# sandeep06011991/OCC-GNN

Measured on AMD Instinct MI355X. Metric: sampled_edges_per_sec, higher is better.
Workload: dtype u32; 1 GPU; products-like synthetic (N=2449029, mean degree 50.5, pareto degrees, seed 0), GraphSAGE fanout 15/10/5 (layer 0 = seeds' hop), minibatch 1024, 4 parts (v % 4), engine-only (sample+slice); streams=128, round_overlap=True, device_lists=int32 (host exports widen to the reference's int64), engine_device_bytes=16549793524

## Files before the change

occ-gnn_amd/csrc/cslicer_hip.hip:

```cpp
#include <hip/hip_runtime.h>

#include <cstdarg>
#include <cstdio>
#include <cstdlib>
#include <cstring>
#include <algorithm>
#include <deque>
#include <vector>

#include "cslicer_hip.h"

namespace {

constexpr uint32_t UNSET = 0xFFFFFFFFu;

constexpr int TN = 256;
#ifdef CSL_OCC7
#define CSL_LB256 __launch_bounds__(256)
#else
#define CSL_LB256 __launch_bounds__(256, 8)
#endif
constexpr int CSL_MAX_SETS = 4;
constexpr int NW = TN / 64;
#ifndef CSL_TPB
#define CSL_TPB 4
#endif
#ifndef CSL_HLOG
#define CSL_HLOG 12
#endif
#ifndef CSL_QMEAN
#define CSL_QMEAN 2048
#endif
#ifndef CSL_SCT
#define CSL_SCT 4096
#endif
#ifndef CSL_SU
#define CSL_SU 1
#endif
constexpr int TPB = CSL_TPB;
constexpr int HLOG = CSL_HLOG;
constexpr int HCAP = 1 << HLOG;
constexpr int QMEAN = CSL_QMEAN;
constexpr int SCT = CSL_SCT;
constexpr int DEG_BITS = 24;
constexpr uint32_t DEG_MASK = (1u << DEG_BITS) - 1;

constexpr int K_NEED = 0;
constexpr int K_EDGES = 1;
constexpr int K_NEWF = 2;
__host__ __device__ constexpr int K_IN(int P, int g) { return 3 + g; }
__host__ __device__ constexpr int K_OUT(int P, int g) { return 3 + P + g; }
__host__ __device__ constexpr int K_OWNED(int P, int g) { return 3 + 2 * P + g; }
__host__ __device__ constexpr int K_SELF(int P, int g) { return 3 + 3 * P + g; }
__host__ __device__ constexpr int K_TO(int P, int g) { return 3 + 4 * P + g; }
__host__ __device__ constexpr int K_FROM(int P, int g) { return 3 + 5 * P + g; }
__host__ __device__ constexpr int K_ECNT(int P, int g) { return 3 + 6 * P + g; }
__host__ __device__ constexpr int K_PAIR(int P, int g, int p) { return 3 + 7 * P + g * P + p; }
__host__ __device__ constexpr int NKINDS(int P, bool graph) { return graph ? 3 + 7 * P + P * P : 3 + 6 * P; }
constexpr int MAXK = 3 + 7 * CSL_MAX_PARTS + CSL_MAX_PARTS * CSL_MAX_PARTS;

enum { KN_SEEDS = 0, KN_DEGREE, KN_SCAN_A, KN_SAMPLE, KN_SCAN_Q, KN_SCATTER, KN_BUCKET, KN_COUNT, KN_SCAN_B,
       KN_EMIT, KN_SELFIN, KN_MT, KN_EDGES, KN_DUPSEEDS, KN_SELFIN_DEGREE };
const char* const kKernelNames[CSL_NUM_KERNELS] = {"k_seeds",   "k_degree", "k_scan_need", "k_sample",
                                                   "k_scan_buckets", "k_scatter", "k_bucket", "k_count",
                                                   "k_scan_lists", "k_emit",  "k_selfin",  "k_mt19937_fill",
                                                   "k_graph", "k_dupseeds", "k_selfin_degree"};

struct LArgs {
  const unsigned long long* rowinfo;
  const uint32_t* off32;
  const uint32_t* indices;
  const uint8_t* wl;
  uint32_t N, P;
  const uint32_t* ring;
  unsigned long long ring_mask, gen_lo, gen_hi;
  unsigned long long* rngpos;
  unsigned long long* rngbase;
  unsigned long long* acc;
  const uint32_t* fr_in;
  uint32_t* fr_out;
  size_t fr_in_stride, fr_out_stride;
  uint32_t fr_out_cap;
  unsigned long long* ninfo;
  uint32_t* hasedge;
  uint32_t* selfpos;
  uint32_t* firstpos;
  size_t fcap;
  uint32_t* cand;
  uint8_t* cflag;
  uint32_t* crank;
  uint2* queue;
  size_t ccap;
  uint32_t* nbk;
  uint32_t* bcnt;
  uint32_t* bcur;
  uint32_t nbmax;
  uint32_t* tcnt;
  uint32_t tmax, nk;
  uint32_t* fsize;
  csl_sample_meta* meta;
  int* arena;
  size_t arena_stride;
  size_t list_base[CSL_NUM_LISTS];
  uint32_t layer, fanout, W;
  unsigned long long wmagic;
  uint32_t S;
  uint32_t tpb;
  uint32_t* boff;
  uint32_t* ticket;
  uint32_t pmagic;
  uint32_t pmask;
  uint32_t last;
  uint32_t* dupflag;
  uint32_t* seedrep;
  uint32_t* dupfirst;
  uint32_t* dupout;
  size_t fcap0;
  unsigned long long* rngend;
  uint32_t* candk;
  uint32_t graph;
  uint8_t* ecnt;
  uint32_t* srcpos;
  uint32_t* tcur;
};

constexpr uint32_t SELF_BIT = 0x80000000u;
constexpr int kNoReplaceMaxFanout = 64;

__device__ __forceinline__ uint32_t mod_parts(const LArgs& a, uint32_t v) {
  uint32_t r = v - __umulhi(v, a.pmagic) * a.P;
  if (r >= a.P) r -= a.P;
  if (r >= a.P) r -= a.P;
  return r;
}
__device__ __forceinline__ uint32_t owner(const LArgs& a, uint32_t v) {
  return a.wl ? (uint32_t)a.wl[v] : mod_parts(a, v);
}
__device__ __forceinline__ unsigned long long row_lookup(const LArgs& a, uint32_t v) {
  if (a.off32) {
    const uint32_t lo = a.off32[v], hi = a.off32[v + 1];
    return ((unsigned long long)lo << 24) | (unsigned long long)(hi - lo);
  }
  return a.rowinfo[v];
}
__device__ __forceinline__ uint32_t lane_id() { return threadIdx.x & 63; }
__device__ __forceinline__ uint32_t div_w(const LArgs& a, uint32_t c) {
  return (uint32_t)(((unsigned long long)c * a.wmagic) >> 40);
}
__device__ __forceinline__ bool xcd_block_at(const LArgs& a, uint32_t id, uint32_t grid, uint32_t& x, uint32_t& s) {
  const uint32_t groups = (a.S + 7u) >> 3;
  const uint32_t per_stream = grid / (8u * groups);
  const uint32_t j = id >> 3;
  const uint32_t sl = j / per_stream;
  x = j - sl * per_stream;
  s = sl * 8u + (id & 7u);
  return s < a.S;
}
__device__ __forceinline__ bool xcd_block(const LArgs& a, uint32_t& x, uint32_t& s) {
  return xcd_block_at(a, blockIdx.x, gridDim.x, x, s);
}
__device__ __forceinline__ void st_sc1(uint32_t* p, uint32_t v) {
  __hip_atomic_store(p, v, __ATOMIC_RELAXED, __HIP_MEMORY_SCOPE_AGENT);
}
__device__ __forceinline__ uint32_t ld_sc1(const uint32_t* p) {
  return __hip_atomic_load(p, __ATOMIC_RELAXED, __HIP_MEMORY_SCOPE_AGENT);
}
__device__ __forceinline__ bool last_block_of_stream(uint32_t* ticket, uint32_t expected) {
  __shared__ uint32_t s_last;
  asm volatile("s_waitcnt vmcnt(0)" ::: "memory");
  __syncthreads();
  if (threadIdx.x == 0) {
    const uint32_t t = __hip_atomic_fetch_add(ticket, 1u, __ATOMIC_RELAXED, __HIP_MEMORY_SCOPE_AGENT);
    s_last = t == expected - 1u;
    if (t == expected - 1u) {
      st_sc1(ticket, 0u);
      __builtin_amdgcn_fence(__ATOMIC_ACQUIRE, "agent");
      asm volatile("s_waitcnt vmcnt(0)" ::: "memory");
    }
  }
  __syncthreads();
  return s_last != 0u;
}
__device__ __forceinline__ unsigned long long lt_mask() {
  return (1ull << lane_id()) - 1ull;
}
__device__ __forceinline__ uint32_t bucket_of(uint32_t v, uint32_t nb) {
  return __umulhi(v * 0x9E3779B1u, nb);
}
__device__ __forceinline__ uint32_t pass_of(uint32_t v, uint32_t npass) {
  uint32_t x = v * 0x27D4EB2Fu;
  x ^= x >> 13;
  return __umulhi(x * 0x165667B1u, npass);
}
__device__ __forceinline__ uint32_t slot_of(uint32_t v) {
  uint32_t x = v * 0x85EBCA6Bu;
  x ^= x >> 15;
  x *= 0xC2B2AE35u;
  return x >> (32 - HLOG);
}

__device__ __forceinline__ uint32_t wave_excl_scan(uint32_t x, uint32_t& total) {
  uint32_t incl = x;
  for (int o = 1; o < 64; o <<= 1) {
    uint32_t y = __shfl_up(incl, o);
    if ((int)lane_id() >= o) incl += y;
  }
  total = __shfl(incl, 63);
  return incl - x;
}

__device__ __forceinline__ uint32_t wave_incl_scan_dpp(uint32_t x) {
  int v = (int)x;
  v += __builtin_amdgcn_update_dpp(0, v, 0x111, 0xf, 0xf, false);
  v += __builtin_amdgcn_update_dpp(0, v, 0x112, 0xf, 0xf, false);
  v += __builtin_amdgcn_update_dpp(0, v, 0x114, 0xf, 0xf, false);
  v += __builtin_amdgcn_update_dpp(0, v, 0x118, 0xf, 0xf, false);
  v += __builtin_amdgcn_update_dpp(0, v, 0x142, 0xa, 0xf, false);
  v += __builtin_amdgcn_update_dpp(0, v, 0x143, 0xc, 0xf, false);
  return (uint32_t)v;
}
__device__ __forceinline__ uint32_t spread4(uint32_t x) { return ((x & 0xFu) * 0x00204081u) & 0x01010101u; }

constexpr int SCAN_CH = 12;

template <int PHASE>
__device__ __forceinline__ void scan_body(const LArgs& a, const int s) {
  const uint32_t F = ld_sc1(&a.fsize[s * (CSL_MAX_LAYERS + 1) + a.layer]);
  const uint32_t ntiles = (F + TN - 1) / TN;
  const int k_lo = PHASE == 0 ? 0 : 2;
  const int k_hi = PHASE == 0 ? 2 : (int)a.nk;
  __shared__ uint32_t s_tot[MAXK];
  const int w = threadIdx.x >> 6, nw = blockDim.x >> 6;
  const uint32_t chunk = (ntiles + 63) / 64;
  for (int k = k_lo + w; k < k_hi; k += nw) {
    uint32_t* p = a.tcnt + ((size_t)s * a.nk + k) * a.tmax;
    if (chunk <= (uint32_t)SCAN_CH) {
      const uint32_t t0 = lane_id() * chunk;
      uint32_t x[SCAN_CH], sum = 0;
#pragma unroll
      for (int j = 0; j < SCAN_CH; j++) {
        x[j] = ((uint32_t)j < chunk && t0 + j < ntiles) ? ld_sc1(&p[t0 + j]) : 0u;
        sum += x[j];
      }
      uint32_t tot;
      uint32_t run = wave_excl_scan(sum, tot);
#pragma unroll
      for (int j = 0; j < SCAN_CH; j++) {
        if ((uint32_t)j < chunk && t0 + j < ntiles) p[t0 + j] = run;
        run += x[j];
      }
      if (lane_id() == 0) s_tot[k] = tot;
    } else {
      uint32_t run = 0;
      for (uint32_t t0 = 0; t0 < ntiles; t0 += 64) {
        const uint32_t t = t0 + lane_id();
        const uint32_t x = t < ntiles ? ld_sc1(&p[t]) : 0;
        uint32_t tot;
        const uint32_t ex = wave_excl_scan(x, tot);
        if (t < ntiles) p[t] = run + ex;
        run += tot;
      }
      if (lane_id() == 0) s_tot[k] = run;
    }
  }
  if (PHASE == 0) {
    const unsigned long long C = (unsigned long long)F * a.W;
    uint32_t nb = (uint32_t)((C + QMEAN - 1) / QMEAN);
    if (nb < 1) nb = 1;
    if (nb > a.nbmax) nb = a.nbmax;
    if (threadIdx.x == 0) a.nbk[s] = F ? nb : 0;
    for (uint32_t b = threadIdx.x; b <= a.nbmax; b += blockDim.x) {
      a.bcnt[(size_t)s * (a.nbmax + 1) + b] = 0;
      if (b < a.nbmax) a.bcur[(size_t)s * a.nbmax + b] = 0;
    }
  }
  __syncthreads();
  csl_layer_meta& m = a.meta[s].layer[a.layer];
  if (PHASE == 0) {
    if (threadIdx.x == 0) {
      const unsigned long long base = a.rngpos[s];
      const unsigned long long draws = (unsigned long long)s_tot[K_NEED] * a.fanout;
      a.rngbase[s] = base;
      a.rngpos[s] = base + draws;
      a.rngend[s] = base + draws;
      if (a.layer == 0) a.meta[s].rng_begin = base;
      a.meta[s].rng_end = base + draws;
      a.acc[2 * s] += s_tot[K_EDGES];
      if (a.layer == 0 && F) a.acc[2 * s + 1] += 1;
      m.frontier = F;
      m.draws = (uint32_t)draws;
      m.sampled_edges = s_tot[K_EDGES];
    }
  } else {
    const int P = (int)a.P;
    const uint32_t t = threadIdx.x;
    auto pair_sum = [&](int g, bool from) -> uint32_t {
      uint32_t x = 0;
      for (int p = 0; p < P; p++) x += from ? s_tot[K_PAIR(P, g, p)] : s_tot[K_PAIR(P, p, g)];
      return x;
    };
    auto tot_of = [&](int kind, int g) -> uint32_t {
      switch (kind) {
        case CSL_IN_NODES: return s_tot[K_IN(P, g)];
        case CSL_OUT_NODES: return s_tot[K_OUT(P, g)];
        case CSL_OWNED_OUT_NODES: return s_tot[K_OWNED(P, g)];
        case CSL_SELF_IDS_IN:
        case CSL_SELF_IDS_OUT: return s_tot[K_SELF(P, g)];
        case CSL_TO_IDS: return a.graph ? pair_sum(g, false) : s_tot[K_TO(P, g)];
        case CSL_FROM_IDS: return a.graph ? pair_sum(g, true) : s_tot[K_FROM(P, g)];
        case CSL_INDPTR: return a.graph ? (F ? s_tot[K_OUT(P, g)] + 1 : 0u) : 0u;
        case CSL_INDICES: return a.graph ? s_tot[K_ECNT(P, g)] : 0u;
        case CSL_T_INDPTR: return a.tcur ? (F ? s_tot[K_IN(P, g)] + 1 : 0u) : 0u;
        case CSL_T_INDICES: return a.tcur ? s_tot[K_ECNT(P, g)] + s_tot[K_SELF(P, g)] : 0u;
        default: return a.graph ? s_tot[K_OWNED(P, g)] : 0u;
      }
    };
    if (t < (uint32_t)CSL_NUM_LISTS) {
      uint32_t run = 0;
      for (int g = 0; g < P; g++) {
        m.off[t][g] = run;
        run += tot_of((int)t, g);
      }
      for (int g = P; g <= CSL_MAX_PARTS; g++) m.off[t][g] = run;
    } else if (t == 16) {
      uint32_t nf = s_tot[K_NEWF];
      if (nf > a.fr_out_cap) {
        atomicOr(&a.meta[s].error, (uint32_t)CSL_ERR_FRONTIER_CAP);
        nf = a.fr_out_cap;
      }
      m.next_frontier = nf;
      a.fsize[s * (CSL_MAX_LAYERS + 1) + a.layer + 1] = nf;
    } else if (t == 17) {
      for (int g = 0; g < CSL_MAX_PARTS; g++)
        m.indptr_len[g] = g < P ? tot_of(a.graph ? CSL_INDPTR : CSL_OUT_NODES, g) : 0u;
    } else if (a.graph && t >= 32 && t < 32u + (uint32_t)P) {
      const int g = (int)t - 32;
      uint32_t fr = 0, to = 0;
      for (int p = 0; p < P; p++) {
        m.pair_off[0][g][p] = fr;
        m.pair_off[1][g][p] = to;
        fr += s_tot[K_PAIR(P, g, p)];
        to += s_tot[K_PAIR(P, p, g)];
      }
      for (int p = P; p <= CSL_MAX_PARTS; p++) {
        m.pair_off[0][g][p] = fr;
        m.pair_off[1][g][p] = to;
      }
    }
  }
}

struct BatchDesc {
  long long offset;
  int count;
  int pad;
};

__device__ __forceinline__ void degree_body(const LArgs& a, const uint32_t bx, const uint32_t s, const uint32_t per_stream,
                                            const long long* __restrict__ nodes, const BatchDesc* __restrict__ desc) {
  uint32_t F;
  long long noff = 0;
  if (a.layer == 0) {
    const BatchDesc d = desc[s];
    F = (uint32_t)d.count;
    noff = d.offset;
    if (bx == 0 && threadIdx.x == 0) {
      st_sc1(&a.fsize[s * (CSL_MAX_LAYERS + 1)], F);
      for (uint32_t l = 1; l <= CSL_MAX_LAYERS; l++) a.fsize[s * (CSL_MAX_LAYERS + 1) + l] = 0;
      a.dupflag[s] = 0;
      a.meta[s].n_seeds = F;
    }
  } else {
    F = a.fsize[s * (CSL_MAX_LAYERS + 1) + a.layer];
  }
  const uint32_t tile = bx * NW + (threadIdx.x >> 6);
  if (tile * TN < F) {
    const uint32_t i0 = tile * TN + lane_id() * 4;
    unsigned long long ri[4] = {0, 0, 0, 0};
    if (a.layer == 0) {
      uint32_t v[4];
#pragma unroll
      for (int j = 0; j < 4; j++) {
        v[j] = UNSET;
        if (i0 + j < F) {
          long long id = nodes[noff + i0 + j];
          if (id < 0 || id >= (long long)a.N) {
            atomicOr(&a.meta[s].error, (uint32_t)CSL_ERR_SEED_RANGE);
            id = 0;
          }
          v[j] = (uint32_t)id;
        }
      }
#pragma unroll
      for (int j = 0; j < 4; j++)
        if (v[j] != UNSET) ri[j] = row_lookup(a, v[j]);
#pragma unroll
      for (int j = 0; j < 4; j++) {
        if (v[j] != UNSET) {
          const_cast<uint32_t*>(a.fr_in)[s * a.fr_in_stride + i0 + j] = v[j];
          a.ninfo[s * a.fcap + i0 + j] = ri[j];
        }
      }
    } else {
#pragma unroll
      for (int j = 0; j < 4; j++)
        if (i0 + j < F) ri[j] = a.ninfo[s * a.fcap + i0 + j];
    }
    uint32_t need = 0, ne = 0;
#pragma unroll
    for (int j = 0; j < 4; j++) {
      if (i0 + j < F) {
        const uint32_t deg = (uint32_t)(ri[j] & DEG_MASK);
        need += deg >= a.fanout;
        ne += deg < a.fanout ? deg : a.fanout;
      }
    }
    for (int o = 32; o > 0; o >>= 1) {
      need += __shfl_down(need, o);
      ne += __shfl_down(ne, o);
    }
    if (lane_id() == 0) {
      st_sc1(&a.tcnt[((size_t)s * a.nk + K_NEED) * a.tmax + tile], need);
      st_sc1(&a.tcnt[((size_t)s * a.nk + K_EDGES) * a.tmax + tile], ne);
    }
  }
  uint32_t nb_act = ((F + TN - 1) / TN + NW - 1) / NW;
  if (nb_act < 1) nb_act = 1;
  if (nb_act > per_stream) nb_act = per_stream;
  if (bx >= nb_act) return;
  if (last_block_of_stream(a.ticket + 2 * s, nb_act)) scan_body<0>(a, (int)s);
}

__global__ CSL_LB256 void k_degree(LArgs a, const long long* __restrict__ nodes,
                                               const BatchDesc* __restrict__ desc) {
  uint32_t bx, s;
  if (!xcd_block(a, bx, s)) return;
  degree_body(a, bx, s, gridDim.x / (8u * ((a.S + 7u) >> 3)), nodes, desc);
}

__device__ __forceinline__ uint32_t mt_temper(uint32_t y) {
  y ^= y >> 11;
  y ^= (y << 7) & 0x9d2c5680u;
  y ^= (y << 15) & 0xefc60000u;
  y ^= y >> 18;
  return y;
}

__device__ __forceinline__ uint32_t ring_word(const LArgs& a, uint32_t s, unsigned long long pos) {
  if (pos >= a.gen_lo && pos < a.gen_hi) return a.ring[pos & a.ring_mask];
  atomicOr(&a.meta[s].error, (uint32_t)CSL_ERR_RNG_WINDOW);
  return 0;
}
__device__ __forceinline__ uint32_t floyd_pick(const LArgs& a, uint32_t s, unsigned long long row_pos, uint32_t j,
                                               uint32_t D, uint32_t rj) {
  uint32_t x = rj % (D + j + 1u);
  const uint32_t own = x;
  uint32_t m = j;
  bool taken = false;
  for (;;) {
    for (uint32_t i = 0; i < m; i++) {
      if (ring_word(a, s, row_pos + i) % (D + i + 1u) == x) taken = true;
    }
    if (taken || x < D || x - D >= m) break;
    m = x - D;
    x = ring_word(a, s, row_pos + m) % (D + m + 1u);
  }
  return taken ? D + j : own;
}

__global__ CSL_LB256 void k_sample(LArgs a) {
  constexpr bool NOREP = false;
  constexpr bool WEIGHTED = false;
  constexpr const uint32_t* cum = nullptr;
#include "k_sample_body.inc"
}
__global__ CSL_LB256 void k_sample_norep(LArgs a) {
  constexpr bool NOREP = true;
  constexpr bool WEIGHTED = false;
  constexpr const uint32_t* cum = nullptr;
#include "k_sample_body.inc"
}
__global__ CSL_LB256 void k_sample_weighted(LArgs a, const uint32_t* __restrict__ cum) {
  constexpr bool NOREP = false;
  constexpr bool WEIGHTED = true;
#include "k_sample_body.inc"
}

__global__ __launch_bounds__(256) void k_check_cdf(const unsigned long long* __restrict__ rowinfo,
// ... 127 lines not shown
  const uint32_t staged = s_loff[nb - 1] + s_hist[nb - 1];
  for (uint32_t k = n; k < staged; k += TN) {
    const uint2 e = s_stage[k];
    const uint32_t b = bucket_of(e.x, nb);
    q[s_gbase[b] + (k - s_loff[b])] = e;
  }
}

__device__ __forceinline__ uint32_t ht_find(const uint32_t* h_key, uint32_t val) {
  uint32_t h = slot_of(val);
  for (uint32_t probes = 0; probes < (uint32_t)HCAP; probes++) {
    const uint32_t k = h_key[h];
    if (k == val) return h;
    if (k == UNSET) return UNSET;
    h = (h + 1) & (HCAP - 1);
  }
  return UNSET;
}

#ifndef CSL_BT
#define CSL_BT 512
#endif
#ifndef CSL_RC
#define CSL_RC 4
#endif
constexpr int BT = CSL_BT;
constexpr int RC = CSL_RC;

__device__ __forceinline__ uint32_t ht_insert(uint32_t* h_key, uint32_t val) {
  uint32_t h = slot_of(val);
  for (uint32_t probes = 0; probes < (uint32_t)HCAP; probes++) {
    uint32_t kk = h_key[h];
    if (kk == UNSET) kk = atomicCAS(&h_key[h], UNSET, val);
    if (kk == UNSET || kk == val) return h;
    h = (h + 1) & (HCAP - 1);
  }
  return UNSET;
}

#ifndef CSL_BPB
#define CSL_BPB 4
#endif
constexpr int BPB = CSL_BPB;

__device__ unsigned long long g_wave_dup[3];

template <bool HAS_WL, bool PROBE = false>
__global__ __launch_bounds__(BT) void k_bucket(LArgs a) {
  uint32_t bx, s;
  if (!xcd_block(a, bx, s)) return;
  const uint32_t nbk = a.nbk[s];
  uint32_t b = bx * BPB;
  if (b >= nbk) return;
  __shared__ __attribute__((aligned(16))) uint32_t h_key[HCAP];
  __shared__ __attribute__((aligned(16))) uint32_t h_epos[HCAP];
  __shared__ __attribute__((aligned(16))) uint32_t h_self[HCAP];
  const uint32_t n = threadIdx.x;
  const uint32_t* off = a.boff + (size_t)s * (a.nbmax + 1);
  const uint2* qs = a.queue + (size_t)s * a.ccap;
  const uint32_t W = a.W;
  uint32_t q0 = off[b], q1 = off[b + 1];
  uint2 e[RC];
#pragma unroll
  for (int r = 0; r < RC; r++) e[r] = n + r * BT < q1 - q0 ? qs[q0 + n + r * BT] : make_uint2(UNSET, 0u);
  auto record = [&](const uint2 ee, const uint32_t h) {
    if (ee.y & SELF_BIT) {
      atomicMin(&h_self[h], ee.y & ~SELF_BIT);
      if (a.graph) atomicMin(&h_epos[h], (ee.y & ~SELF_BIT) * W);
    } else {
      atomicMin(&h_epos[h], ee.y);
    }
  };
  auto insert = [&](const uint2 ee) -> uint32_t {
    const uint32_t h = ht_insert(h_key, ee.x);
    if (h == UNSET) {
      atomicOr(&a.meta[s].error, (uint32_t)CSL_ERR_BUCKET_FULL);
    } else {
      record(ee, h);
    }
    return h;
  };
  uint8_t* cflag = a.cflag + (size_t)s * a.ccap;
  auto part_of = [&](const uint32_t v) -> uint32_t { return HAS_WL ? (uint32_t)a.wl[v] : mod_parts(a, v); };
  auto judge = [&](const uint2 ee, const uint32_t epos, const uint32_t self, const uint32_t g) {
    if (ee.y & SELF_BIT) {
      const uint32_t i = ee.y & ~SELF_BIT;
      const uint32_t c = i * W;
      if (self != i) {
        if (a.graph) atomicOr(&a.meta[s].error, (uint32_t)CSL_ERR_DUP_SEED);
        else a.dupflag[s] = 1u;
      }
      if (a.graph) {
        const uint32_t fe = epos == c;
        if (!fe) cflag[c] = 0;
        a.firstpos[s * a.fcap + i] = epos;
      } else {
        const uint32_t newf = epos > c && self == i;
        if (!newf) cflag[c] = 0;
        if (a.layer == 0) a.seedrep[s * a.fcap0 + i] = self;
        if (epos != UNSET) a.firstpos[s * a.fcap + i] = epos;
      }
    } else {
      const uint32_t c = ee.y;
      const uint32_t fe = epos == c;
      if (!fe) {
        cflag[c] = 0;
      } else if (!a.graph && self != UNSET) {
        const uint32_t newf = (unsigned long long)self * W > c;
        cflag[c] = (uint8_t)(newf | 2u | (g << 2) | 32u);
      }
      if (a.graph && !fe) a.srcpos[(size_t)s * a.ccap + c] = epos;
    }
  };
  auto evaluate = [&](const uint2 ee, const uint32_t h) { judge(ee, h_epos[h], h_self[h], part_of(ee.x)); };
  for (int j = 0; j < BPB; j++, b++) {
    if (b >= nbk) break;
    const uint2* q = qs + q0;
    const uint32_t cnt = q1 - q0;
    if (PROBE) {
      unsigned n_e = 0, n_row = 0, n_all = 0;
      const uint32_t lane = lane_id();
#pragma unroll
      for (int r = 0; r < RC; r++) {
        bool later_row = false, later_all = false;
        for (uint32_t sl = 0; sl < 64; sl++) {
#pragma unroll
          for (int r2 = 0; r2 < RC; r2++) {
            const uint32_t other = __shfl(e[r2].x, sl);
            if (other == e[r].x && (r2 < r || (r2 == r && sl < lane))) {
              later_all = true;
              if (r2 == r) later_row = true;
            }
          }
        }
        if (e[r].x != UNSET) {
          n_e++;
          n_row += later_row;
          n_all += later_all;
        }
      }
      atomicAdd(&g_wave_dup[0], (unsigned long long)n_e);
      atomicAdd(&g_wave_dup[1], (unsigned long long)n_row);
      atomicAdd(&g_wave_dup[2], (unsigned long long)n_all);
    }
    uint2 en[RC];
    const bool more = j + 1 < BPB && b + 1 < nbk;
    const uint32_t q1n = off[more ? b + 2 : b + 1];
#pragma unroll
    for (int r = 0; r < RC; r++) {
      const uint32_t k = n + r * BT;
      const bool ok = more && k < q1n - q1;
      en[r] = qs[ok ? q1 + k : 0u];
      if (!ok) en[r] = make_uint2(UNSET, 0u);
    }
    auto clear_table = [&]() {
      const uint4 u4 = make_uint4(UNSET, UNSET, UNSET, UNSET);
      for (uint32_t i = n; i < (uint32_t)HCAP / 4; i += BT) {
        reinterpret_cast<uint4*>(h_key)[i] = u4;
        reinterpret_cast<uint4*>(h_epos)[i] = u4;
        reinterpret_cast<uint4*>(h_self)[i] = u4;
      }
    };
    if (cnt > (uint32_t)HCAP) {
      const uint32_t npass = (cnt + (uint32_t)HCAP / 2 - 1) / ((uint32_t)HCAP / 2);
      for (uint32_t pass = 0; pass < npass; pass++) {
        clear_table();
        __syncthreads();
        for (uint32_t k = n; k < cnt; k += BT) {
          const uint2 ee = q[k];
          if (pass_of(ee.x, npass) == pass) insert(ee);
        }
        __syncthreads();
        for (uint32_t k = n; k < cnt; k += BT) {
          const uint2 ee = q[k];
          if (pass_of(ee.x, npass) != pass) continue;
          const uint32_t h = ht_find(h_key, ee.x);
          if (h != UNSET) evaluate(ee, h);
        }
        __syncthreads();
      }
    } else {
    clear_table();
    __syncthreads();
    uint32_t hs[RC];
#pragma unroll
    for (int r = 0; r < RC; r++) hs[r] = e[r].x != UNSET ? insert(e[r]) : UNSET;
    for (uint32_t k = n + RC * BT; k < cnt; k += BT) insert(q[k]);
    __syncthreads();
    {
      uint32_t og[RC], ep[RC], sf[RC];
#pragma unroll
      for (int r = 0; r < RC; r++) {
        og[r] = hs[r] != UNSET ? part_of(e[r].x) : 0u;
        ep[r] = hs[r] != UNSET ? h_epos[hs[r]] : UNSET;
        sf[r] = hs[r] != UNSET ? h_self[hs[r]] : UNSET;
      }
#pragma unroll
      for (int r = 0; r < RC; r++)
        if (hs[r] != UNSET) judge(e[r], ep[r], sf[r], og[r]);
    }
    for (uint32_t k = n + RC * BT; k < cnt; k += BT) {
      const uint2 ee = q[k];
      const uint32_t h = ht_find(h_key, ee.x);
      if (h != UNSET) evaluate(ee, h);
    }
    }
    if (!more) break;
    __syncthreads();
#pragma unroll
    for (int r = 0; r < RC; r++) e[r] = en[r];
    q0 = q1;
    q1 = q1n;
  }
}

__device__ __forceinline__ void count_tile(const LArgs& a, const uint32_t s, const uint32_t tile, const uint32_t F);

constexpr int CNT_T = 1024;
__global__ __launch_bounds__(CNT_T) void k_count(LArgs a) {
  uint32_t bx, s;
  if (!xcd_block(a, bx, s)) return;
  const uint32_t F = a.fsize[s * (CSL_MAX_LAYERS + 1) + a.layer];
  const uint32_t tile = bx * (CNT_T / 64) + (threadIdx.x >> 6);
  if (tile * TN < F) count_tile(a, s, tile, F);
  const uint32_t per_stream = gridDim.x / (8u * ((a.S + 7u) >> 3));
  uint32_t nb_act = ((F + TN - 1) / TN + CNT_T / 64 - 1) / (CNT_T / 64);
  if (nb_act < 1) nb_act = 1;
  if (nb_act > per_stream) nb_act = per_stream;
  if (bx >= nb_act) return;
  if (last_block_of_stream(a.ticket + 2 * s + 1, nb_act)) scan_body<1>(a, (int)s);
}

__device__ __forceinline__ void count_tile(const LArgs& a, const uint32_t s, const uint32_t tile, const uint32_t F) {
  const uint32_t W = a.W, P = a.P;
  const uint32_t nodes_here = (F - tile * TN) < (uint32_t)TN ? (F - tile * TN) : (uint32_t)TN;
  const uint32_t nbytes = nodes_here * W;
  const uint32_t* fw = reinterpret_cast<const uint32_t*>(a.cflag + (size_t)s * a.ccap + (size_t)tile * TN * W);
  uint32_t c_new = 0;
  unsigned long long acc_lo = 0, acc_hi = 0;
  for (uint32_t o = lane_id() * 4; o < nbytes; o += 256) {
    uint32_t w = fw[o >> 2];
    if (o + 4 > nbytes) w &= 0xFFFFFFFFu >> (8 * (o + 4 - nbytes));
    c_new += __popc(w & 0x01010101u);
#pragma unroll
    for (int b = 0; b < 4; b++) {
      const uint32_t fl = (w >> (8 * b)) & 0xFFu;
      const unsigned long long one = (unsigned long long)((fl >> 1) & 1u) << (16u * ((fl >> 2) & 3u));
      if (P > 4 && (fl & 16u)) acc_hi += one; else acc_lo += one;
    }
  }
  uint32_t cnt[1 + CSL_MAX_PARTS];
  if (nbytes < 65536u) {
    for (int o = 32; o > 0; o >>= 1) {
      c_new += __shfl_down(c_new, o);
      acc_lo += __shfl_down(acc_lo, o);
      if (P > 4) acc_hi += __shfl_down(acc_hi, o);
    }
    cnt[0] = c_new;
#pragma unroll
    for (int g = 0; g < 4; g++) {
      cnt[1 + g] = (uint32_t)(acc_lo >> (16 * g)) & 0xFFFFu;
      cnt[5 + g] = (uint32_t)(acc_hi >> (16 * g)) & 0xFFFFu;
    }
  } else {
    cnt[0] = c_new;
#pragma unroll
    for (int g = 0; g < 4; g++) {
      cnt[1 + g] = (uint32_t)(acc_lo >> (16 * g)) & 0xFFFFu;
      cnt[5 + g] = (uint32_t)(acc_hi >> (16 * g)) & 0xFFFFu;
    }
#pragma unroll
    for (int k = 0; k < 1 + CSL_MAX_PARTS; k++) {
      uint32_t x = cnt[k];
      for (int o = 32; o > 0; o >>= 1) x += __shfl_down(x, o);
      cnt[k] = x;
    }
  }
  if (lane_id() == 0) {
#pragma unroll
    for (int k = 0; k < 1 + CSL_MAX_PARTS; k++)
      if (k < 1 + (int)P) st_sc1(&a.tcnt[((size_t)s * a.nk + (K_NEWF + k)) * a.tmax + tile], cnt[k]);
  }
}

#ifndef CSL_EP
#define CSL_EP 8
#endif
constexpr int EP = CSL_EP;

__global__ CSL_LB256 void k_emit(LArgs a) {
  uint32_t tile, s;
  if (!xcd_block(a, tile, s)) return;
  const uint32_t F = a.fsize[s * (CSL_MAX_LAYERS + 1) + a.layer];
  if (tile * TN >= F) return;
  const uint32_t n = threadIdx.x;
  const uint32_t w = __builtin_amdgcn_readfirstlane(n >> 6);
  const uint32_t lane = lane_id();
  const uint32_t W = a.W, P = a.P;
  const csl_layer_meta& m = a.meta[s].layer[a.layer];
  int* ar = a.arena + (size_t)s * a.arena_stride;
  const uint32_t* tc = a.tcnt + (size_t)s * a.nk * a.tmax;
#define TB(kind) tc[(size_t)(kind)*a.tmax + tile]
  static_assert(NW == 4, "four wave counts per word");
  __shared__ uint32_t s_wc[2][1 + CSL_MAX_PARTS];
  __shared__ uint32_t s_run[2][1 + CSL_MAX_PARTS];
  __shared__ uint32_t s_wn[5 * 2 * NW];
  const uint32_t below = (1u << (8u * w)) - 1u;
#define WBYTE(word) (reinterpret_cast<uint8_t*>(&(word))[w])
#define BYTESUM(x) __builtin_amdgcn_sad_u8((x), 0u, 0u)
  __shared__ uint32_t s_tb[5 * CSL_MAX_PARTS];
  __shared__ uint32_t s_mo[6][CSL_MAX_PARTS];
  if (n < 1 + P) s_run[0][n] = n == 0 ? TB(K_NEWF) : TB(K_IN(P, n - 1));
  if (n >= 64 && n < 64 + 5 * P) s_tb[n - 64] = TB(K_OUT(P, 0) + (n - 64));
  if (n >= 128 && n < 128 + 6 * CSL_MAX_PARTS) {
    const uint32_t k6 = (n - 128) / CSL_MAX_PARTS, g = (n - 128) % CSL_MAX_PARTS;
    const int list = k6 == 0 ? CSL_IN_NODES : k6 == 1 ? CSL_OUT_NODES : k6 == 2 ? CSL_OWNED_OUT_NODES
                   : k6 == 3 ? CSL_SELF_IDS_OUT : k6 == 4 ? CSL_TO_IDS : CSL_FROM_IDS;
    s_mo[k6][g] = g < P ? m.off[list][g] : 0u;
  }
  const uint32_t i = tile * TN + n;
  const bool act = i < F;
  uint32_t v = 0, hb = 0;
  if (act) {
    v = a.fr_in[s * a.fr_in_stride + i];
    hb = a.hasedge[s * a.fcap + i];
  }
  const uint32_t nodes_here = (F - tile * TN) < (uint32_t)TN ? (F - tile * TN) : (uint32_t)TN;
  const uint32_t ncand = nodes_here * W;
  const uint32_t iters = (ncand + TN - 1) / TN;
  const size_t cbase = (size_t)s * a.ccap + (size_t)tile * TN * W;
  const uint32_t nf_cap = m.next_frontier;
  const unsigned long long lt = lt_mask();
  uint32_t* fr_out = a.fr_out + s * a.fr_out_stride;
  unsigned long long* ninfo = a.ninfo + s * a.fcap;
  int* in_list = ar + a.list_base[CSL_IN_NODES];
  const uint8_t* __restrict__ cflag = a.cflag;
  const uint32_t* __restrict__ cand = a.cand;
  for (uint32_t c0 = 0; c0 < iters; c0 += EP) {
    uint32_t pf[EP], pv[EP];
#pragma unroll
    for (int j = 0; j < EP; j++) {
      const uint32_t k = (c0 + j) * TN + n;
      pf[j] = k < ncand ? cflag[cbase + k] : 0u;
      pv[j] = k < ncand ? cand[cbase + k] : 0u;
    }
#pragma unroll
    for (int j = 0; j < EP; j++) {
      if (c0 + j >= iters) break;
      const uint32_t b = j & 1;
      const uint32_t fl = pf[j], val = pv[j];
      const uint32_t newf = fl & 1u, fe = (fl >> 1) & 1u, g = (fl >> 2) & 7u;
      const unsigned long long m0 = __ballot(newf);
      const uint32_t r0 = __popcll(m0 & lt);
      uint32_t rE = 0;
      if (lane == 0) WBYTE(s_wc[b][0]) = (uint8_t)__popcll(m0);
#pragma unroll
      for (uint32_t gg = 0; gg < CSL_MAX_PARTS; gg++) {
        if (gg < P) {
          const unsigned long long mg = __ballot(fe && g == gg);
          if (g == gg) rE = __popcll(mg & lt);
          if (lane == 0) WBYTE(s_wc[b][1 + gg]) = (uint8_t)__popcll(mg);
        }
      }
      __syncthreads();
      if (n < 1 + P) s_run[b ^ 1][n] = s_run[b][n] + BYTESUM(s_wc[b][n]);
      if (newf) {
        const uint32_t p = s_run[b][0] + r0 + BYTESUM(s_wc[b][0] & below);
        if (p < nf_cap) {
          fr_out[p] = val;
          if (!a.last) ninfo[p] = row_lookup(a, val);
        }
      }
#ifndef CSL_ABLATE_EMIT_IN
      if (fe && ((a.pmask >> g) & 1u)) {
        const uint32_t p = s_run[b][1 + g] + rE + BYTESUM(s_wc[b][1 + g] & below);
        in_list[s_mo[0][g] + p] = (int)val;
        if (a.tcur) a.tcur[(size_t)s * a.ccap + s_mo[0][g] + p] = 0;
        if (a.graph || (fl & 32u)) a.crank[cbase + (c0 + j) * TN + n] = p;
      }
#endif
    }
  }
  static_assert(EP % 2 == 0, "buffer parity");
  const uint32_t to = act ? owner(a, v) : 0u;
  const uint32_t ob = act ? 1u << to : 0u;
  const uint32_t oth = hb & ~ob;
  const bool hi = P > 4;
  const uint32_t one_to = act ? 1u << (8u * (to & 3u)) : 0u;
  const bool to_hi = to >= 4;
  uint32_t wd[5][2];
  wd[0][0] = spread4(hb);
  wd[4][0] = spread4(oth);
  wd[1][0] = (!to_hi && (hb & ob)) ? one_to : 0u;
  wd[2][0] = !to_hi ? one_to : 0u;
  wd[3][0] = (!to_hi && oth) ? one_to : 0u;
  wd[0][1] = wd[1][1] = wd[2][1] = wd[3][1] = wd[4][1] = 0;
  if (hi) {
    wd[0][1] = spread4(hb >> 4);
    wd[4][1] = spread4(oth >> 4);
    wd[1][1] = (to_hi && (hb & ob)) ? one_to : 0u;
    wd[2][1] = to_hi ? one_to : 0u;
    wd[3][1] = (to_hi && oth) ? one_to : 0u;
  }
#pragma unroll
  for (int k = 0; k < 5; k++) {
#pragma unroll
    for (int h = 0; h < 2; h++) {
      if (h == 0 || hi) {
        const uint32_t incl = wave_incl_scan_dpp(wd[k][h]);
        if (lane == 63) s_wn[(k * 2 + h) * NW + w] = incl;
        wd[k][h] = incl - wd[k][h];
      }
    }
  }
  __syncthreads();
  const uint32_t m0 = w > 0 ? 0xFFFFFFFFu : 0u, m1 = w > 1 ? 0xFFFFFFFFu : 0u, m2 = w > 2 ? 0xFFFFFFFFu : 0u;
#pragma unroll
  for (int k = 0; k < 5; k++) {
#pragma unroll
    for (int h = 0; h < 2; h++) {
      if (h == 0 || hi) {
        const uint32_t* c = &s_wn[(k * 2 + h) * NW];
        wd[k][h] += (c[0] & m0) + (c[1] & m1) + (c[2] & m2);
      }
    }
  }
#define RANK(k, g) ((wd[k][(g) >> 2] >> (8u * ((g)&3u))) & 0xFFu)
#ifndef CSL_ABLATE_EMIT_NODES
  if (act) {
    int outrank_to = -1;
#pragma unroll
    for (uint32_t g = 0; g < CSL_MAX_PARTS; g++) {
      if (g < P && ((hb >> g) & 1u)) {
        const uint32_t p = RANK(0, g) + s_tb[0 * P + g];
        if (g == to) outrank_to = p;
        if (!((a.pmask >> g) & 1u)) continue;
        ar[a.list_base[CSL_OUT_NODES] + s_mo[1][g] + p] = (int)v;
        if (g != to && !a.graph) {
          const uint32_t q = RANK(4, g) + s_tb[4 * P + g];
          ar[a.list_base[CSL_FROM_IDS] + s_mo[5][g] + q] = (int)p;
        }
      }
    }
    const uint32_t tsh = 8u * (to & 3u);
#define RANK_TO(k) (((to_hi ? wd[k][1] : wd[k][0]) >> tsh) & 0xFFu)
    const bool mine = (a.pmask >> to) & 1u;
    {
      const uint32_t q = RANK_TO(2) + s_tb[2 * P + to];
      const uint32_t pos = s_mo[3][to] + q;
      if (mine) ar[a.list_base[CSL_SELF_IDS_OUT] + pos] = outrank_to;
      a.selfpos[s * a.fcap + i] = mine ? pos : UNSET;
    }
    if (outrank_to >= 0 && mine) {
      const uint32_t q = RANK_TO(1) + s_tb[1 * P + to];
      ar[a.list_base[CSL_OWNED_OUT_NODES] + s_mo[2][to] + q] = outrank_to;
    }
    if (!a.graph && oth != 0 && mine) {
      const uint32_t q = RANK_TO(3) + s_tb[3 * P + to];
      ar[a.list_base[CSL_TO_IDS] + s_mo[4][to] + q] = outrank_to;
    }
#undef RANK_TO
  }
#else
  if (act) a.selfpos[s * a.fcap + i] = 0;
#endif
#undef RANK
#undef TB
#undef WBYTE
#undef BYTESUM
}

constexpr int DS_T = 256;
__device__ __forceinline__ uint32_t ds_ld(const uint32_t* p) {
  return __hip_atomic_load(p, __ATOMIC_RELAXED, __HIP_MEMORY_SCOPE_AGENT);
}
template <bool IS_MAX>
__device__ __forceinline__ uint32_t ds_block_scan(uint32_t x, uint32_t* s_w, uint32_t& total) {
  const uint32_t lane = lane_id(), w = threadIdx.x >> 6;
  uint32_t incl = x;
  for (int o = 1; o < 64; o <<= 1) {
    const uint32_t y = __shfl_up(incl, o);
    if ((int)lane >= o) incl = IS_MAX ? (incl > y ? incl : y) : incl + y;
  }
  uint32_t excl = __shfl_up(incl, 1);
  if (lane == 0) excl = 0;
  __syncthreads();
  if (lane == 63) s_w[w] = incl;
  __syncthreads();
  uint32_t before = 0, all = 0;
  for (uint32_t k = 0; k < DS_T / 64; k++) {
    const uint32_t t = s_w[k];
    if (k < w) before = IS_MAX ? (before > t ? before : t) : before + t;
    all = IS_MAX ? (all > t ? all : t) : all + t;
  }
  total = all;
  return IS_MAX ? (excl > before ? excl : before) : excl + before;
}

__global__ __launch_bounds__(DS_T) void k_dupseeds(LArgs a) {
  const uint32_t s = blockIdx.x;
  if (!a.dupflag[s]) return;
  const uint32_t F = a.fsize[s * (CSL_MAX_LAYERS + 1)], P = a.P, n = threadIdx.x;
  const uint32_t* fr = a.fr_in + s * a.fr_in_stride;
  const uint32_t* hbv = a.hasedge + s * a.fcap;
  const uint32_t* rep = a.seedrep + s * a.fcap0;
  uint32_t* firstg = a.dupfirst + (size_t)s * a.fcap0 * P;
  uint32_t* outidx = a.dupout + (size_t)s * a.fcap0 * P;
  uint32_t* selfpos = a.selfpos + s * a.fcap;
  int* ar = a.arena + (size_t)s * a.arena_stride;
  csl_layer_meta& m = a.meta[s].layer[0];
  __shared__ uint32_t s_w[DS_T / 64];
  __shared__ uint32_t s_cnt[6][CSL_MAX_PARTS];
  __shared__ uint32_t s_off[5][CSL_MAX_PARTS + 1];
  for (uint32_t k = n; k < F * P; k += DS_T) firstg[k] = UNSET;
  __syncthreads();
  for (uint32_t i = n; i < F; i += DS_T) {
    const uint32_t h = hbv[i], r = rep[i];
    for (uint32_t g = 0; g < P; g++)
      if ((h >> g) & 1u) atomicMin(&firstg[(size_t)r * P + g], i);
  }
  __syncthreads();
  const uint32_t chunks = (F + DS_T - 1) / DS_T;
  for (int pass = 0; pass < 2; pass++) {
    for (uint32_t g = 0; g < P; g++) {
      for (int kind = pass == 0 ? 0 : 1; kind < (pass == 0 ? 6 : 5); kind++) {
        uint32_t run = 0, prev_run = 0;
        for (uint32_t ch = 0; ch < chunks; ch++) {
          const uint32_t i = ch * DS_T + n;
          const bool act = i < F;
          uint32_t v = 0, h = 0, r = 0, to = 0;
          if (act) {
            v = fr[i];
            h = hbv[i];
            r = rep[i];
            to = owner(a, v);
          }
          const bool bit = act && ((h >> g) & 1u), own = act && to == g;
          bool mem;
          if (kind == 0) mem = bit && ds_ld(&firstg[(size_t)r * P + g]) == i;
          else if (kind == 1) mem = own && bit;
          else if (kind == 2) mem = own;
          else if (kind == 3) mem = own && (h & ~(1u << g)) != 0;
          else if (kind == 4) mem = bit && !own;
          else mem = bit;
          if (kind != 0) {
            uint32_t tot;
            uint32_t pm = ds_block_scan<true>(mem ? i + 1 : 0u, s_w, tot);
            if (pm < prev_run) pm = prev_run;
            if (tot > prev_run) prev_run = tot;
            if (mem && pm != 0 && rep[pm - 1] == r) mem = false;
          }
          uint32_t tot;
          const uint32_t rank = run + ds_block_scan<false>(mem ? 1u : 0u, s_w, tot);
          run += tot;
          if (pass == 0) {
            if (kind == 0 && mem) outidx[(size_t)i * P + g] = rank;
          } else if (act) {
            const uint32_t fo = ds_ld(&firstg[(size_t)r * P + g]);
            const int oi = fo == UNSET ? -1 : (int)ds_ld(&outidx[(size_t)fo * P + g]);
            if (kind == 1 && mem) ar[a.list_base[CSL_OWNED_OUT_NODES] + s_off[1][g] + rank] = oi;
            if (kind == 2) {
              if (mem) ar[a.list_base[CSL_SELF_IDS_OUT] + s_off[2][g] + rank] = oi;
              if (own) selfpos[i] = mem ? s_off[2][g] + rank : UNSET;
            }
            if (kind == 3 && mem) ar[a.list_base[CSL_TO_IDS] + s_off[3][g] + rank] = oi;
            if (kind == 4 && mem) ar[a.list_base[CSL_FROM_IDS] + s_off[4][g] + rank] = oi;
          }
        }
        if (pass == 0 && n == 0) s_cnt[kind][g] = run;
      }
    }
    __syncthreads();
    if (pass == 0) {
      if (n < 5) {
        uint32_t run = 0;
        for (uint32_t g = 0; g <= CSL_MAX_PARTS; g++) {
          s_off[n][g] = run;
          if (g < P) run += s_cnt[n][g];
        }
        const int list = n == 0 ? CSL_OUT_NODES : n == 1 ? CSL_OWNED_OUT_NODES : n == 2 ? CSL_SELF_IDS_OUT
                       : n == 3 ? CSL_TO_IDS : CSL_FROM_IDS;
        for (uint32_t g = 0; g <= CSL_MAX_PARTS; g++) {
          m.off[list][g] = s_off[n][g];
          if (n == 2) m.off[CSL_SELF_IDS_IN][g] = s_off[n][g];
        }
      }
      if (n >= 64 && n < 64 + P) m.indptr_len[n - 64] = s_cnt[5][n - 64];
      __syncthreads();
      for (uint32_t i = n; i < F; i += DS_T) {
        const uint32_t v = fr[i], h = hbv[i], r = rep[i];
        for (uint32_t g = 0; g < P; g++)
          if (((h >> g) & 1u) && ds_ld(&firstg[(size_t)r * P + g]) == i)
            ar[a.list_base[CSL_OUT_NODES] + s_off[0][g] + ds_ld(&outidx[(size_t)i * P + g])] = (int)v;
      }
      __syncthreads();
    }
  }
}

__global__ __launch_bounds__(TN) void k_graph(LArgs a) {
  uint32_t tile, s;
  if (!xcd_block(a, tile, s)) return;
  const uint32_t F = a.fsize[s * (CSL_MAX_LAYERS + 1) + a.layer];
  if (tile * TN >= F) return;
  const uint32_t n = threadIdx.x, w = n >> 6;
  const uint32_t W = a.W, P = a.P;
  const csl_layer_meta& m = a.meta[s].layer[a.layer];
  int* ar = a.arena + (size_t)s * a.arena_stride;
  const uint32_t* tc = a.tcnt + (size_t)s * a.nk * a.tmax;
#define TB(kind) tc[(size_t)(kind)*a.tmax + tile]
  __shared__ uint32_t s_wo[NW][CSL_MAX_PARTS];
  __shared__ uint32_t s_we[NW][CSL_MAX_PARTS];
  __shared__ uint32_t s_wp[NW][CSL_MAX_PARTS * CSL_MAX_PARTS];
  const uint32_t i = tile * TN + n;
  const bool act = i < F;
  uint32_t v = 0, hb = 0, to = 0;
  if (act) {
    v = a.fr_in[s * a.fr_in_stride + i];
    hb = a.hasedge[s * a.fcap + i];
    to = owner(a, v);
  }
  uint32_t r_out[CSL_MAX_PARTS], ec[CSL_MAX_PARTS], r_ec[CSL_MAX_PARTS], r_pair[CSL_MAX_PARTS];
  const unsigned long long lt = lt_mask();
#pragma unroll
  for (uint32_t g = 0; g < CSL_MAX_PARTS; g++) {
    r_out[g] = ec[g] = r_ec[g] = r_pair[g] = 0;
    if (g < P) {
      const bool has = act && ((hb >> g) & 1u);
      const unsigned long long b_out = __ballot(has);
      r_out[g] = __popcll(b_out & lt);
      ec[g] = act ? (uint32_t)a.ecnt[(s * a.fcap + i) * P + g] : 0u;
      uint32_t tot;
      r_ec[g] = wave_excl_scan(ec[g], tot);
      if (lane_id() == 0) {
        s_wo[w][g] = __popcll(b_out);
        s_we[w][g] = tot;
      }
      for (uint32_t p = 0; p < P; p++) {
        const unsigned long long b_pair = __ballot(has && to == p && p != g);
        if (to == p) r_pair[g] = __popcll(b_pair & lt);
        if (lane_id() == 0) s_wp[w][g * CSL_MAX_PARTS + p] = __popcll(b_pair);
      }
    }
  }
  __syncthreads();
  if (!act) return;
  uint32_t outrank[CSL_MAX_PARTS], rs[CSL_MAX_PARTS];
  uint32_t deg = 0;
#pragma unroll
  for (uint32_t g = 0; g < CSL_MAX_PARTS; g++) {
    outrank[g] = rs[g] = 0;
    if (g < P) {
      uint32_t p = r_out[g], q = r_ec[g];
      for (uint32_t ww = 0; ww < w; ww++) {
        p += s_wo[ww][g];
        q += s_we[ww][g];
      }
      outrank[g] = p + TB(K_OUT(P, g));
      rs[g] = q + TB(K_ECNT(P, g));
      deg += ec[g];
      if (((hb >> g) & 1u) && ((a.pmask >> g) & 1u))
        ar[a.list_base[CSL_INDPTR] + m.off[CSL_INDPTR][g] + outrank[g] + 1] = (int)(rs[g] + ec[g]);
      if (i == 0) ar[a.list_base[CSL_INDPTR] + m.off[CSL_INDPTR][g]] = 0;
    }
  }
#pragma unroll
  for (uint32_t g = 0; g < CSL_MAX_PARTS; g++) {
    if (g < P && g != to && ((hb >> g) & 1u)) {
      uint32_t q = r_pair[g];
      for (uint32_t ww = 0; ww < w; ww++) q += s_wp[ww][g * CSL_MAX_PARTS + to];
      q += TB(K_PAIR(P, g, to));
      if ((a.pmask >> g) & 1u)
        ar[a.list_base[CSL_FROM_IDS] + m.off[CSL_FROM_IDS][g] + m.pair_off[0][g][to] + q] = (int)outrank[g];
      if ((a.pmask >> to) & 1u)
        ar[a.list_base[CSL_TO_IDS] + m.off[CSL_TO_IDS][to] + m.pair_off[1][to][g] + q] = (int)outrank[to];
    }
  }
  if ((a.pmask >> to) & 1u) {
    const uint32_t q = a.selfpos[s * a.fcap + i] - m.off[CSL_SELF_IDS_OUT][to];
    ar[a.list_base[CSL_OWNED_DEGREE] + m.off[CSL_OWNED_DEGREE][to] + q] = (int)deg;
  }
  const size_t cb = (size_t)s * a.ccap + (size_t)i * W;
  for (uint32_t slot = 1; slot < W; slot++) {
    const uint32_t val = a.cand[cb + slot];
    if (val == UNSET) continue;
    const uint32_t g = owner(a, val);
    if (!((a.pmask >> g) & 1u)) continue;
// ... 1539 lines not shown
```

Baseline: 31.28 billion edges/s.

## Batch emit ranks per EP chunk with two barriers and batched row lookups

Restructures k_emit so each chunk of EP candidate rows computes its wave ballots first, then does a single block-level prefix over all EP rows, cutting the per-row __syncthreads to two per chunk. Row-info lookups for new frontier nodes are issued in groups of four before their stores, so several loads are in flight at once. Loads become unconditional with clamped indices, flag bytes are packed into words, popcount ranks use mbcnt, and the owner lookup is hoisted into the first chunk and kept in shared memory. The cost is more shared memory and registers per thread, which could lower occupancy.

```diff
diff --git a/occ-gnn_amd/csrc/cslicer_hip.hip b/occ-gnn_amd/csrc/cslicer_hip.hip
--- a/occ-gnn_amd/csrc/cslicer_hip.hip
+++ b/occ-gnn_amd/csrc/cslicer_hip.hip
@@ -184,6 +184,9 @@
 __device__ __forceinline__ unsigned long long lt_mask() {
   return (1ull << lane_id()) - 1ull;
 }
+__device__ __forceinline__ uint32_t rank_below(unsigned long long m) {
+  return __builtin_amdgcn_mbcnt_hi((uint32_t)(m >> 32), __builtin_amdgcn_mbcnt_lo((uint32_t)m, 0u));
+}
 __device__ __forceinline__ uint32_t bucket_of(uint32_t v, uint32_t nb) {
   return __umulhi(v * 0x9E3779B1u, nb);
 }
@@ -917,15 +920,16 @@
   const uint32_t* tc = a.tcnt + (size_t)s * a.nk * a.tmax;
 #define TB(kind) tc[(size_t)(kind)*a.tmax + tile]
   static_assert(NW == 4, "four wave counts per word");
-  __shared__ uint32_t s_wc[2][1 + CSL_MAX_PARTS];
-  __shared__ uint32_t s_run[2][1 + CSL_MAX_PARTS];
+  __shared__ uint32_t s_wc[2][EP][1 + CSL_MAX_PARTS];
+  __shared__ uint32_t s_base[2][EP][1 + CSL_MAX_PARTS];
   __shared__ uint32_t s_wn[5 * 2 * NW];
+  __shared__ uint8_t s_to[TN];
   const uint32_t below = (1u << (8u * w)) - 1u;
 #define WBYTE(word) (reinterpret_cast<uint8_t*>(&(word))[w])
 #define BYTESUM(x) __builtin_amdgcn_sad_u8((x), 0u, 0u)
   __shared__ uint32_t s_tb[5 * CSL_MAX_PARTS];
   __shared__ uint32_t s_mo[6][CSL_MAX_PARTS];
-  if (n < 1 + P) s_run[0][n] = n == 0 ? TB(K_NEWF) : TB(K_IN(P, n - 1));
+  if (n < 1 + P) s_base[0][0][n] = n == 0 ? TB(K_NEWF) : TB(K_IN(P, n - 1));
   if (n >= 64 && n < 64 + 5 * P) s_tb[n - 64] = TB(K_OUT(P, 0) + (n - 64));
   if (n >= 128 && n < 128 + 6 * CSL_MAX_PARTS) {
     const uint32_t k6 = (n - 128) / CSL_MAX_PARTS, g = (n - 128) % CSL_MAX_PARTS;
@@ -935,69 +939,132 @@
   }
   const uint32_t i = tile * TN + n;
   const bool act = i < F;
-  uint32_t v = 0, hb = 0;
-  if (act) {
-    v = a.fr_in[s * a.fr_in_stride + i];
-    hb = a.hasedge[s * a.fcap + i];
-  }
+  uint32_t v = a.fr_in[s * a.fr_in_stride + (act ? i : tile * TN)];
+  uint32_t hb = a.hasedge[s * a.fcap + (act ? i : tile * TN)];
+  if (!act) v = hb = 0;
   const uint32_t nodes_here = (F - tile * TN) < (uint32_t)TN ? (F - tile * TN) : (uint32_t)TN;
   const uint32_t ncand = nodes_here * W;
   const uint32_t iters = (ncand + TN - 1) / TN;
   const size_t cbase = (size_t)s * a.ccap + (size_t)tile * TN * W;
   const uint32_t nf_cap = m.next_frontier;
-  const unsigned long long lt = lt_mask();
   uint32_t* fr_out = a.fr_out + s * a.fr_out_stride;
   unsigned long long* ninfo = a.ninfo + s * a.fcap;
   int* in_list = ar + a.list_base[CSL_IN_NODES];
   const uint8_t* __restrict__ cflag = a.cflag;
   const uint32_t* __restrict__ cand = a.cand;
-  for (uint32_t c0 = 0; c0 < iters; c0 += EP) {
-    uint32_t pf[EP], pv[EP];
+  uint32_t c0 = 0;
+  do {
+    uint32_t pv[EP], pfb[EP];
 #pragma unroll
     for (int j = 0; j < EP; j++) {
       const uint32_t k = (c0 + j) * TN + n;
-      pf[j] = k < ncand ? cflag[cbase + k] : 0u;
-      pv[j] = k < ncand ? cand[cbase + k] : 0u;
+      pv[j] = cand[cbase + (k < ncand ? k : 0u)];
     }
 #pragma unroll
     for (int j = 0; j < EP; j++) {
-      if (c0 + j >= iters) break;
-      const uint32_t b = j & 1;
-      const uint32_t fl = pf[j], val = pv[j];
+      const uint32_t k = (c0 + j) * TN + n;
+      pfb[j] = cflag[cbase + (k < ncand ? k : 0u)];
+    }
+    uint32_t pf[EP / 4];
+#pragma unroll
+    for (int j = 0; j < EP; j++) {
+      const uint32_t k = (c0 + j) * TN + n;
+      const uint32_t f = (k < ncand ? pfb[j] : 0u) << (8 * (j & 3));
+      pf[j >> 2] = (j & 3) ? pf[j >> 2] | f : f;
+    }
+#define PF(j) ((pf[(j) >> 2] >> (8 * ((j)&3))) & 0xFFu)
+    uint32_t own = 0;
+    if (c0 == 0 && act) own = owner(a, v);
+    const uint32_t cp = (c0 / EP) & 1u;
+    uint32_t rk[EP / 2];
+#pragma unroll
+    for (int j = 0; j < EP; j++) {
+      if (!(j & 1)) rk[j >> 1] = 0;
+      if (c0 + j >= iters) continue;
+      const uint32_t fl = PF(j);
       const uint32_t newf = fl & 1u, fe = (fl >> 1) & 1u, g = (fl >> 2) & 7u;
       const unsigned long long m0 = __ballot(newf);
-      const uint32_t r0 = __popcll(m0 & lt);
+      const uint32_t r0 = rank_below(m0);
       uint32_t rE = 0;
-      if (lane == 0) WBYTE(s_wc[b][0]) = (uint8_t)__popcll(m0);
+      if (lane == 0) WBYTE(s_wc[cp][j][0]) = (uint8_t)__popcll(m0);
 #pragma unroll
       for (uint32_t gg = 0; gg < CSL_MAX_PARTS; gg++) {
         if (gg < P) {
           const unsigned long long mg = __ballot(fe && g == gg);
-          if (g == gg) rE = __popcll(mg & lt);
-          if (lane == 0) WBYTE(s_wc[b][1 + gg]) = (uint8_t)__popcll(mg);
+          if (g == gg) rE = rank_below(mg);
+          if (lane == 0) WBYTE(s_wc[cp][j][1 + gg]) = (uint8_t)__popcll(mg);
         }
       }
-      __syncthreads();
-      if (n < 1 + P) s_run[b ^ 1][n] = s_run[b][n] + BYTESUM(s_wc[b][n]);
-      if (newf) {
-        const uint32_t p = s_run[b][0] + r0 + BYTESUM(s_wc[b][0] & below);
-        if (p < nf_cap) {
-          fr_out[p] = val;
-          if (!a.last) ninfo[p] = row_lookup(a, val);
+      rk[j >> 1] |= (r0 | (rE << 8)) << (16 * (j & 1));
+    }
+    __syncthreads();
+    if (n < 1 + P) {
+      uint32_t base = s_base[cp][0][n];
+#pragma unroll
+      for (int j = 0; j < EP; j++) {
+        if (c0 + j >= iters) break;
+        if (j) s_base[cp][j][n] = base;
+        base += BYTESUM(s_wc[cp][j][n]);
+      }
+      s_base[cp ^ 1u][0][n] = base;
+    }
+    __syncthreads();
+#define POS_NEW(j) (s_base[cp][j][0] + BYTESUM(s_wc[cp][j][0] & below) + ((rk[(j) >> 1] >> (16 * ((j)&1))) & 0xFFu))
+#define POS_IN(j, g) \
+  (s_base[cp][j][1 + (g)] + BYTESUM(s_wc[cp][j][1 + (g)] & below) + ((rk[(j) >> 1] >> (16 * ((j)&1) + 8)) & 0xFFu))
+    if (c0 == 0) s_to[n] = (uint8_t)own;
+    uint32_t nfm = 0;
+#pragma unroll
+    for (int j = 0; j < EP; j++)
+      if ((PF(j) & 1u) && POS_NEW(j) < nf_cap) nfm |= 1u << j;
+    if (!a.last) {
+      constexpr int LK = 4;
+#pragma unroll
+      for (int j0 = 0; j0 < EP; j0 += LK) {
+        if (c0 + j0 >= iters) break;
+        uint32_t n0[LK], n1[LK];
+#pragma unroll
+        for (int t = 0; t < LK; t++) {
+          const uint32_t vj = (nfm >> (j0 + t)) & 1u ? pv[j0 + t] : 0u;
+          if (a.off32) {
+            n0[t] = a.off32[vj];
+            n1[t] = a.off32[vj + 1];
+          } else {
+            const uint2 ri = reinterpret_cast<const uint2*>(a.rowinfo)[vj];
+            n0[t] = ri.x;
+            n1[t] = ri.y;
+          }
         }
-      }
+#pragma unroll
+        for (int t = 0; t < LK; t++) asm volatile("" ::"v"(n0[t]), "v"(n1[t]));
+#pragma unroll
+        for (int t = 0; t < LK; t++) {
+          if ((nfm >> (j0 + t)) & 1u)
+            ninfo[POS_NEW(j0 + t)] =
+                a.off32 ? ((unsigned long long)n0[t] << 24) | (unsigned long long)(n1[t] - n0[t])
+                        : ((unsigned long long)n1[t] << 32) | n0[t];
+        }
+      }
+    }
+#pragma unroll
+    for (int j = 0; j < EP; j++) {
+      const uint32_t val = pv[j], fl = PF(j), g = (fl >> 2) & 7u;
+      if ((nfm >> j) & 1u) fr_out[POS_NEW(j)] = val;
 #ifndef CSL_ABLATE_EMIT_IN
-      if (fe && ((a.pmask >> g) & 1u)) {
-        const uint32_t p = s_run[b][1 + g] + rE + BYTESUM(s_wc[b][1 + g] & below);
+      if ((fl & 2u) && ((a.pmask >> g) & 1u)) {
+        const uint32_t p = POS_IN(j, g);
         in_list[s_mo[0][g] + p] = (int)val;
         if (a.tcur) a.tcur[(size_t)s * a.ccap + s_mo[0][g] + p] = 0;
         if (a.graph || (fl & 32u)) a.crank[cbase + (c0 + j) * TN + n] = p;
       }
 #endif
     }
-  }
-  static_assert(EP % 2 == 0, "buffer parity");
-  const uint32_t to = act ? owner(a, v) : 0u;
+#undef POS_NEW
+#undef POS_IN
+  } while ((c0 += EP) < iters);
+#undef PF
+  static_assert(EP % 4 == 0, "four flag bytes per word");
+  const uint32_t to = s_to[n];
   const uint32_t ob = act ? 1u << to : 0u;
   const uint32_t oth = hb & ~ob;
   const bool hi = P > 4;
```

Result: no change. 31.50 billion edges/s (median of 6 runs) (+0.7%).
